# OpenVVC/OpenVVC

Hardware: AMD Instinct MI355X
Metric: decoded frames/sec, full rcn back-end decode step (H2D of the recorded picture + MC incl. BDOF/DMVR/affine-PROF/GPM/CIIP + LMCS + inverse transform + ordered intra pass + deblocking + SAO + ALF/CC-ALF + D2H of refined MVs + wait + per-picture digest + publication to the device DPB), 4K 10-bit RA rec (higher is better)
Workload: dtype u16 samples / int16 coefficients / int32 accumulate

## Files before the change

### openvvc_amd/csrc/kernels_mcx.hip

```cpp
#include "mc_common.hip.h"

#ifndef OV_WPE_MCX
#define OV_WPE_MCX 4
#endif
#if OV_WPE_MCX > 0
#define OV_OCC_MCX __attribute__((amdgpu_waves_per_eu(OV_WPE_MCX)))
#else
#define OV_OCC_MCX
#endif

namespace {

#define XWIN_STRIDE  32
#define XCWIN_STRIDE 20
#define XWIN_ROWS    28
#define XCWIN_ROWS   16
#define BIL_STRIDE   20
#define R_STRIDE     18

__device__ __forceinline__ void clip_mv_dev(int px, int py, int pic_w, int pic_h, int pw, int ph, int &mvx, int &mvy)
{
    mvx = ov_clip3(mvx, -((pw + 3 + px) << 4), (pic_w + 2 - px) << 4);
    mvy = ov_clip3(mvy, -((ph + 3 + py) << 4), (pic_h + 2 - py) << 4);
}

__device__ __forceinline__ void pad_sides(uint16_t *win, int stride, int ww, int wh, int lane)
{
    if (lane < wh) {
        uint16_t *r = win + lane * stride;
        const uint16_t a = r[0], b = r[ww - 1];
        r[-1] = a; r[-2] = a; r[ww] = b; r[ww + 1] = b;
    }
}
__device__ __forceinline__ void pad_rows(uint16_t *win, int stride, int ww, int wh, int lane)
{
    if (lane < ww + 4) {
        uint16_t *c = win + lane - 2;
        const uint16_t a = c[0], b = c[(wh - 1) * stride];
        c[-stride] = a; c[-2 * stride] = a; c[wh * stride] = b; c[(wh + 1) * stride] = b;
    }
}

template <int ND>
__device__ __forceinline__ uint32_t sad_row(const int *a, const int *b, bool odd, uint32_t acc)
{
    uint32_t A[ND + 1], B[ND + 1];
#pragma unroll
    for (int k = 0; k < ND + 1; ++k) { A[k] = (uint32_t)a[k]; B[k] = (uint32_t)b[k]; }
    if (odd) {
#pragma unroll
        for (int k = 0; k < ND; ++k) {
            A[k] = __builtin_amdgcn_alignbit(A[k + 1], A[k], 16);
            B[k] = __builtin_amdgcn_alignbit(B[k + 1], B[k], 16);
        }
    }
#pragma unroll
    for (int k = 0; k < ND; ++k) acc = __builtin_amdgcn_sad_u16(A[k], B[k], acc);
    return acc;
}

__device__ __forceinline__ int div_for_maxq7(int num, int den)
{
    int sign = 0, q = 0;
    if (num < 0) { sign = 1; num = -num; }
    den <<= 3;
    if (num >= den) { num -= den; q++; }
    q <<= 1; den >>= 1;
    if (num >= den) { num -= den; q++; }
    q <<= 1;
    if (num >= (den >> 1)) q++;
    return sign ? -q : q;
}

#define MCX_LDS_WL (2 * XWIN_ROWS * XWIN_STRIDE * 2)
#define MCX_LDS_WC (4 * XCWIN_ROWS * XCWIN_STRIDE * 2)
#define MCX_LDS    (MCX_LDS_WL + MCX_LDS_WC + (2 * 16 * HT_STRIDE + 4 * 8 * CHT_STRIDE) * 2)

template <bool SEARCH_ONLY>
__device__ __forceinline__ void mcx_units(const ovhip_pic &dst, const RefTable &refs, const ovhip_mc_unit *__restrict__ units,
                                          uint32_t n_units, const uint16_t *__restrict__ lmcs_fwd, int32_t *__restrict__ mv_out,
                                          uint32_t wg, char *lds)
{
    uint16_t (*const s_wl)[XWIN_ROWS * XWIN_STRIDE] = reinterpret_cast<uint16_t (*)[XWIN_ROWS * XWIN_STRIDE]>(lds);
    uint16_t (*const s_wc)[2][XCWIN_ROWS * XCWIN_STRIDE] =
        reinterpret_cast<uint16_t (*)[2][XCWIN_ROWS * XCWIN_STRIDE]>(lds + MCX_LDS_WL);
    int16_t *const s_h = reinterpret_cast<int16_t *>(lds + MCX_LDS_WL + MCX_LDS_WC);
    int16_t (*const s_hl)[16 * HT_STRIDE] = reinterpret_cast<int16_t (*)[16 * HT_STRIDE]>(s_h);
    int16_t (*const s_hc)[2][8 * CHT_STRIDE] = reinterpret_cast<int16_t (*)[2][8 * CHT_STRIDE]>(s_h + 2 * 16 * HT_STRIDE);
    int16_t (*const s_x)[24 * BIL_STRIDE] = reinterpret_cast<int16_t (*)[24 * BIL_STRIDE]>(s_h);
    static_assert(2 * 24 * BIL_STRIDE <= 2 * 16 * HT_STRIDE + 4 * 8 * CHT_STRIDE, "bilinear blocks must fit the H tiles");
    uint32_t *const s_ba = reinterpret_cast<uint32_t *>(s_wl[0]);
    uint32_t *const s_bb = s_ba + 256;
    int16_t  *const s_bc = reinterpret_cast<int16_t *>(s_bb + 256);
    static_assert(2 * XWIN_ROWS * XWIN_STRIDE * 2 >= 2 * 1024 + 512, "BDOF terms must fit the luma windows");

    const int lane = threadIdx.x;
    {
    if (wg >= n_units) return;
    const uint32_t bid = ov_xcd_slot(wg, n_units);
    const ovhip_mc_unit u = units[bid];
    const bool dmvr = u.flags & OVHIP_MC_DMVR;
    if (SEARCH_ONLY && !dmvr) return;
    bool use_bdof = u.flags & OVHIP_MC_BDOF;
    const bool do_l = !(u.flags & OVHIP_MC_NO_LUMA), do_c = !(u.flags & OVHIP_MC_NO_CHROMA);
    const int w = u.w, h = u.h, wc = w >> 1, hc = h >> 1;
    const int log2w = 31 - __clz(w), log2wc = log2w - 1;

    int mv[2][2] = { { u.mv0x, u.mv0y }, { u.mv1x, u.mv1y } };
    int ini[2][2] = { { u.mv0x, u.mv0y }, { u.mv1x, u.mv1y } };

    uint16_t *wl[2], *wcp[2][2];
    int offl[2], offc[2];
    {
        const uint16_t *const ry[2]  = { refs.p[u.ref0].y,  refs.p[u.ref1].y };
        const uint16_t *const rcb[2] = { refs.p[u.ref0].cb, refs.p[u.ref1].cb };
        const uint16_t *const rcr[2] = { refs.p[u.ref0].cr, refs.p[u.ref1].cr };
        int lx[2], ly[2], cx[2], cy[2];
#pragma unroll
        for (int l = 0; l < 2; ++l) {
            int ax = mv[l][0], ay = mv[l][1];
            if (dmvr) clip_mv_dev(u.x, u.y, dst.w, dst.h, w, h, ax, ay);
            lx[l] = u.x + (ax >> 4) - 3;        ly[l] = u.y + (ay >> 4) - 3;
            cx[l] = (u.x >> 1) + (ax >> 5) - 1; cy[l] = (u.y >> 1) + (ay >> 5) - 1;
        }
        uint16_t *const lwin[2] = { s_wl[0] + 2 * XWIN_STRIDE + 4, s_wl[1] + 2 * XWIN_STRIDE + 4 };
        uint16_t *const cwin[4] = { s_wc[0][0] + 2 * XCWIN_STRIDE + 4, s_wc[0][1] + 2 * XCWIN_STRIDE + 4,
                                    s_wc[1][0] + 2 * XCWIN_STRIDE + 4, s_wc[1][1] + 2 * XCWIN_STRIDE + 4 };
        stage_unit_windows(dst, ry, rcb, rcr, lx, ly, cx, cy, w, h, 3, do_l, do_c, lane, lwin, XWIN_STRIDE, cwin, XCWIN_STRIDE, offl, offc);
#pragma unroll
        for (int l = 0; l < 2; ++l) {
            wl[l] = lwin[l] + offl[l];
            wcp[0][l] = cwin[l] + offc[l]; wcp[1][l] = cwin[2 + l] + offc[l];
        }
    }
    __syncthreads();

    if (dmvr) {
#pragma unroll
        for (int l = 0; l < 2; ++l) {
            if (do_l) pad_sides(wl[l], XWIN_STRIDE, w + 7, h + 7, lane);
            if (do_c) { pad_sides(wcp[0][l], XCWIN_STRIDE, wc + 3, hc + 3, lane); pad_sides(wcp[1][l], XCWIN_STRIDE, wc + 3, hc + 3, lane); }
        }
        __syncthreads();
#pragma unroll
        for (int l = 0; l < 2; ++l) {
            if (do_l) pad_rows(wl[l], XWIN_STRIDE, w + 7, h + 7, lane);
            if (do_c) { pad_rows(wcp[0][l], XCWIN_STRIDE, wc + 3, hc + 3, lane); pad_rows(wcp[1][l], XCWIN_STRIDE, wc + 3, hc + 3, lane); }
        }
        {
            const int l = lane >= 32, i = lane & 31;
            if (i <= w + 4) {
                const int fx = ini[l][0] & 15, fy = ini[l][1] & 15;
                const uint16_t *src = wl[l] + XWIN_STRIDE + i + 1;
                int16_t *o = s_x[l] + i;
                int tp = 0;
                for (int j = 0; j < h + 5; ++j) {
                    const int a = src[j * XWIN_STRIDE];
                    const int b = __builtin_amdgcn_update_dpp(0, a, 0x130 , 0xf, 0xf, false);
                    const int t = fx ? (__mul24(16 - fx, a) + __mul24(fx, b) + 8) >> 4 : a;
                    if (j && i < w + 4) o[(j - 1) * BIL_STRIDE] = (int16_t)(fy ? (__mul24(16 - fy, tp) + __mul24(fy, t) + 8) >> 4 : tp);
                    tp = t;
                }
            }
        }
        __syncthreads();
        int sad = 0;
        {
            const int k = lane < 25 ? lane : lane - 25, half = lane >= 25;
            if (lane < 50) {
                const int dx = k % 5 - 2, dy = k / 5 - 2;
                const int c0 = 2 + dx, c1 = 2 - dx;
                const bool odd = c0 & 1;
                const int *r0 = reinterpret_cast<const int *>(s_x[0] + (2 + dy) * BIL_STRIDE) + (c0 >> 1);
                const int *r1 = reinterpret_cast<const int *>(s_x[1] + (2 - dy) * BIL_STRIDE) + (c1 >> 1);
                const int nrow = h >> 2;
                uint32_t acc = 0;
                for (int jj = 0; jj < nrow; ++jj) {
                    const int ro = 2 * (half * nrow + jj) * (BIL_STRIDE / 2);
                    if (w == 16) acc = sad_row<8>(r0 + ro, r1 + ro, odd, acc);
                    else         acc = sad_row<4>(r0 + ro, r1 + ro, odd, acc);
                }
// ... 16 lines not shown
            const int s2 = __shfl(sad, max(idx - 5, 0)), s4 = __shfl(sad, min(idx + 5, 24));
            if (abs(dh) != 32 && abs(dv) != 32) {
                const int den_h = s1 + s3 - 2 * s0, den_v = s2 + s4 - 2 * s0;
                if (den_h) dh += (s1 != s0 && s3 != s0) ? div_for_maxq7((s1 - s3) << 4, den_h) : (s1 == s0 ? -8 : 8);
                if (den_v) dv += (s2 != s0 && s4 != s0) ? div_for_maxq7((s2 - s4) << 4, den_v) : (s2 == s0 ? -8 : 8);
            }
            dh = __builtin_amdgcn_readfirstlane(dh); dv = __builtin_amdgcn_readfirstlane(dv);
            mv[0][0] = ov_clip3(mv[0][0] + dh, -(1 << 17), (1 << 17) - 1); mv[0][1] = ov_clip3(mv[0][1] + dv, -(1 << 17), (1 << 17) - 1);
            mv[1][0] = ov_clip3(mv[1][0] - dh, -(1 << 17), (1 << 17) - 1); mv[1][1] = ov_clip3(mv[1][1] - dv, -(1 << 17), (1 << 17) - 1);
        }
        min_cost = __builtin_amdgcn_readfirstlane(min_cost);
        if (use_bdof && min_cost < 2 * w * h) use_bdof = false;
        __syncthreads();
    }
    if (mv_out && lane == 0) {
        int4 o; o.x = mv[0][0]; o.y = mv[0][1]; o.z = mv[1][0]; o.w = mv[1][1];
        *reinterpret_cast<int4 *>(mv_out + 4 * (size_t)bid) = o;
    }
    if (SEARCH_ONLY) return;

    const uint32_t *fvl[2];
    int ldx[2], ldy[2], cdx[2], cdy[2], ext[2][2];
    int fxs[2];
#pragma unroll
    for (int l = 0; l < 2; ++l) {
        int fx = mv[l][0] & 15, fy = mv[l][1] & 15;
        if (u.flags & OVHIP_MC_HPEL_FILT) { if (fx == 8) fx = 16; if (fy == 8) fy = 16; }
        ext[l][0] = fx >= 8; ext[l][1] = fy >= 8;
        fvl[l] = g_taps.luma[fy];
        ldx[l] = (mv[l][0] >> 4) - (ini[l][0] >> 4); ldy[l] = (mv[l][1] >> 4) - (ini[l][1] >> 4);
        cdx[l] = (mv[l][0] >> 5) - (ini[l][0] >> 5); cdy[l] = (mv[l][1] >> 5) - (ini[l][1] >> 5);
        fxs[l] = fx;
    }
    const int hfx = (lane >> 5) ? fxs[1] : fxs[0], hfc = ((lane >> 4) & 1 ? mv[1][0] : mv[0][0]) & 31;
    const uint4 hl_tp = *reinterpret_cast<const uint4 *>(g_taps.luma[hfx]);
    const uint2 hc_tp = *reinterpret_cast<const uint2 *>(g_taps.chroma[hfc]);
    if (do_l) {
        const int l = lane >> 5;
        const int tp[4] = { (int)hl_tp.x, (int)hl_tp.y, (int)hl_tp.z, (int)hl_tp.w };
        const uint16_t *src = s_wl[0] + l * (XWIN_ROWS * XWIN_STRIDE) + (2 + (l ? ldy[1] : ldy[0])) * XWIN_STRIDE;
        const int off = 4 + (l ? offl[1] + ldx[1] : offl[0] + ldx[0]);
        h_pass<8>(src, XWIN_STRIDE, off, h + 7, log2w - 2, 5, lane & 31, tp, hfx == 0, s_hl[0] + l * 16 * HT_STRIDE, HT_STRIDE);
    }
    if (do_c) {
        const int qi = lane >> 4, l = qi & 1;
        const int tp[2] = { (int)hc_tp.x, (int)hc_tp.y };
        const uint16_t *src = s_wc[0][0] + qi * (XCWIN_ROWS * XCWIN_STRIDE) + (2 + (l ? cdy[1] : cdy[0])) * XCWIN_STRIDE;
        const int off = 4 + (l ? offc[1] + cdx[1] : offc[0] + cdx[0]);
        h_pass<4>(src, XCWIN_STRIDE, off, hc + 3, log2wc > 2 ? log2wc - 2 : 0, 4, lane & 15, tp, hfc == 0, s_hc[0][0] + qi * 8 * CHT_STRIDE,
                  CHT_STRIDE);
    }
    __syncthreads();

    if (do_l) {
        int P[2][4];
        v_pass<8>(s_hl[0], HT_STRIDE, log2w, h, fvl[0], lane, P[0]);
        v_pass<8>(s_hl[1], HT_STRIDE, log2w, h, fvl[1], lane, P[1]);
        const bool act = lane < ((h >> 2) << log2w);
        const int x = lane & (w - 1), g = lane >> log2w;
        int out[4];
        if (use_bdof) {
            if (act) {
#pragma unroll
                for (int l = 0; l < 2; ++l)
#pragma unroll
                    for (int j = 0; j < 4; ++j) s_x[l][(4 * g + j + 1) * R_STRIDE + x + 1] = (int16_t)P[l][j];
            }
            const int nring = 2 * (w + 2) + 2 * h;
            for (int t = lane; t < 2 * nring; t += 64) {
                const int l = t >= nring, e = l ? t - nring : t;
                int i, j;
                if (e < w + 2)            { i = e; j = 0; }
                else if (e < 2 * (w + 2)) { i = e - (w + 2); j = h + 1; }
                else if (e < 2 * (w + 2) + h) { i = 0; j = e - 2 * (w + 2) + 1; }
                else                      { i = w + 1; j = e - 2 * (w + 2) - h + 1; }
                const uint16_t *sp = wl[l] + (3 + ldy[l] + j - 1 + ext[l][1]) * XWIN_STRIDE + 3 + ldx[l] + i - 1 + ext[l][0];
                s_x[l][j * R_STRIDE + i] = (int16_t)(*sp << 4);
            }
            __syncthreads();
            int dgx[4], dgy[4];
            if (act) {
                int col[2][6];
#pragma unroll
// ... 34 lines not shown
                        b2 += __builtin_bit_cast(bd_s2, s_bb[idx]);
                        s_dy += s_bc[idx];
                    }
                }
                int s_ax = (unsigned short)a2.x, s_ay = (unsigned short)a2.y, s_xy = b2.x, s_dx = b2.y;
#pragma unroll
                for (int m = 1; m < 4; m <<= 1) {
                    s_ax += __shfl_xor(s_ax, m); s_ay += __shfl_xor(s_ay, m); s_xy += __shfl_xor(s_xy, m);
                    s_dx += __shfl_xor(s_dx, m); s_dy += __shfl_xor(s_dy, m);
                }
                if (s_ax) wx = ov_clip3((s_dx * 4) >> (31 - __clz(s_ax)), -15, 15);
                if (s_ay) {
                    const int x_off = wx ? (wx * s_xy) >> 1 : 0;
                    wy = ov_clip3(((s_dy * 4) - x_off) >> (31 - __clz(s_ay)), -15, 15);
                }
            }
#pragma unroll
            for (int j = 0; j < 4; ++j) out[j] = ov_clip_bd((int)(int16_t)((P[0][j] + P[1][j] + __mul24(wx, dgx[j]) + __mul24(wy, dgy[j]) + 16) >> 5));
        } else {
#pragma unroll
            for (int j = 0; j < 4; ++j) out[j] = ov_clip_bd((P[0][j] + P[1][j] + 16) >> 5);
        }
        if (act) {
            uint16_t *d = dst.y + ov_rowoff(u.y + 4 * g, dst.stride_y) + u.x + x;
#pragma unroll
            for (int j = 0; j < 4; ++j) {
                int v = out[j];
                if ((u.flags & OVHIP_MC_LMCS) && lmcs_fwd) v = lmcs_fwd[v];
                d[j * dst.stride_y] = (uint16_t)v;
            }
        }
    }
    if (do_c) {
        int tvc[2][2];
        load_taps<2>(g_taps.chroma[mv[0][1] & 31], tvc[0]); load_taps<2>(g_taps.chroma[mv[1][1] & 31], tvc[1]);
        if (wc * hc >= 64) chroma_finish<2, true>(u, dst, s_hc[0][0], tvc, lane, log2wc, hc, dst);
        else               chroma_finish<1, true>(u, dst, s_hc[0][0], tvc, lane, log2wc, hc, dst);
    }
    __syncthreads();
    }
}

}


namespace {

#define AWS AFF_WS
#define AHS 12
#define ACS AFF_WS
#define ACHS 8

#ifdef OV_MCA_PHASES
#define OV_MCA_PHASE_UNITS 65536
__device__ unsigned int g_mca_phase[OV_MCA_PHASE_UNITS * 8];
#define OV_APHASE(i) do { __builtin_amdgcn_s_waitcnt(0); const unsigned long long t_ = __builtin_readcyclecounter(); \
                          ph[i] = (unsigned int)(t_ - tprev); tprev = t_; } while (0)
#else
#define OV_APHASE(i) do { } while (0)
#endif

#define MCA_LDS_WIN  (16 * 9 * AWS * 2)
#define MCA_LDS_HT   (16 * 4 * AHS * 2)
#define MCA_LDS_T    (16 * 40 * 2)
#define MCA_LDS_CWIN (2 * 8 * 7 * ACS * 2)
#define MCA_LDS      (MCA_LDS_WIN + MCA_LDS_HT + MCA_LDS_T + MCA_LDS_CWIN + 2 * 8 * 4 * ACHS * 2)

__device__ __forceinline__ void mca_units(const ovhip_pic &dst, const RefTable &refs, const ovhip_aff_unit *__restrict__ units,
                                          uint32_t n_units, const int32_t *__restrict__ side, const uint16_t *__restrict__ lmcs_fwd,
                                          uint32_t wg, char *lds)
{
    uint16_t (*const s_win)[9 * AWS] = reinterpret_cast<uint16_t (*)[9 * AWS]>(lds);
    int16_t  (*const s_ht)[4 * AHS]  = reinterpret_cast<int16_t (*)[4 * AHS]>(lds + MCA_LDS_WIN);
    int16_t  (*const s_t)[40]        = reinterpret_cast<int16_t (*)[40]>(lds + MCA_LDS_WIN + MCA_LDS_HT);
    uint16_t (*const s_cwin)[8][7 * ACS] = reinterpret_cast<uint16_t (*)[8][7 * ACS]>(lds + MCA_LDS_WIN + MCA_LDS_HT + MCA_LDS_T);
    int16_t  (*const s_cht)[8][4 * ACHS] = reinterpret_cast<int16_t (*)[8][4 * ACHS]>(lds + MCA_LDS_WIN + MCA_LDS_HT + MCA_LDS_T + MCA_LDS_CWIN);

    const int lane = threadIdx.x;
    {
    if (wg >= n_units) return;
    const uint32_t bid = ov_xcd_slot(wg, n_units);
#ifdef OV_MCA_PHASES
    unsigned int ph[8] = {}; unsigned long long tprev = __builtin_readcyclecounter();
#endif
    const ovhip_aff_unit u = units[bid];
    OV_APHASE(0);
    const int nsx = u.w >> 2, nsb = nsx * (u.h >> 2), ncx = u.w >> 3, ncb = ncx * (u.h >> 3);
    const bool do_c = !(u.flags & OVHIP_AFF_NO_CHROMA);
    const int4 *mvs = reinterpret_cast<const int4 *>(side + u.side_off);

    const int sb = lane >> 2, c = lane & 3;
    const bool act = sb < nsb;
    const int bx = u.x + 4 * (sb % nsx), by = u.y + 4 * (sb / nsx);
    int4 m = make_int4(0, 0, 0, 0);
    if (act) m = mvs[sb];
    const int cl = lane >> 5, cwi = (lane >> 2) & 7, cblk = cwi & 3, ccomp = cwi >> 2, cc = lane & 3;
    const bool cact = do_c && cblk < ncb && (u.dir & (1 << cl));
    int4 cm = make_int4(0, 0, 0, 0);
    if (do_c && cblk < ncb) cm = mvs[nsb + cblk];
    const int cbx = (u.x >> 1) + 4 * (cblk % ncx), cby = (u.y >> 1) + 4 * (cblk / ncx);
    int coff = 0;

    OV_APHASE(1);

    AffStage<9> st;
    const int rsy = dst.stride_y, rpw = dst.w, rph = dst.h;
    const int lfirst = (u.dir & 1) ? 0 : 1;
    if (act) {
        const int mvx = lfirst ? m.z : m.x, mvy = lfirst ? m.w : m.y;
        st.issue(refs.p[lfirst ? u.ref1 : u.ref0].y, rsy, rpw, rph, bx + (mvx >> 4) - 2, by + (mvy >> 4) - 2, c);
    }
    if (cact) {
        const ovhip_pic &rp = refs.p[cl ? u.ref1 : u.ref0];
        const int mvx = cl ? cm.z : cm.x, mvy = cl ? cm.w : cm.y;
        AffStage<7> cst;
        cst.issue(ccomp ? rp.cr : rp.cb, rp.stride_c, rp.w >> 1, rp.h >> 1, cbx + (mvx >> 5) - 1, cby + (mvy >> 5) - 1, cc);
        coff = cst.park(rp.stride_c, rp.w >> 1, rp.h >> 1, cc, s_cwin[cl][cwi]);
    }
    bool prof[2];
    int pdx[2][4], pdy[2][4];
#pragma unroll
    for (int l = 0; l < 2; ++l) {
        prof[l] = act && (u.dir & (1 << l)) && (u.flags & OVHIP_AFF_PROF) && (u.dir != 3 || ((u.prof_dir >> l) & 1));
        if (prof[l]) {
            const int16_t *pt = reinterpret_cast<const int16_t *>(side + u.prof_off) + 32 * l;
#pragma unroll
            for (int j = 0; j < 4; ++j) { pdx[l][j] = pt[4 * j + c]; pdy[l][j] = pt[16 + 4 * j + c]; }
        }
    }
    OV_APHASE(2);

    int P[2][4] = { { 0, 0, 0, 0 }, { 0, 0, 0, 0 } };
#pragma unroll
    for (int l = 0; l < 2; ++l) {
        const bool on = (u.dir & (1 << l)) && act;
        const int mvx = l ? m.z : m.x, mvy = l ? m.w : m.y;
        int off = 0;
        if (l) __syncthreads();
        if (on) off = st.park(rsy, rpw, rph, c, s_win[sb]);
        if (l == 0 && u.dir == 3 && act)
            st.issue(refs.p[u.ref1].y, rsy, rpw, rph, bx + (m.z >> 4) - 2, by + (m.w >> 4) - 2, c);
        __syncthreads();
        if (on) {
            int tp[3];
            load_taps<3>(g_taps.luma6[mvx & 15], tp);
            for (int r = c; r < 9; r += 4) {
                int d[5], out[4];
                load_row_at<6>(s_win[sb] + r * AWS, off, d);
                fir4<6>(d, tp, out);
#pragma unroll
                for (int o = 0; o < 4; ++o) s_ht[sb][o * AHS + r] = (int16_t)(out[o] >> (OV_BD - 8));
            }
        }
        if (l == 0 && cact) {
            const int cmvx = cl ? cm.z : cm.x;
            int tp[2];
            load_taps<2>(g_taps.chroma[cmvx & 31], tp);
            for (int r = cc; r < 7; r += 4) {
                int d[4], out[4];
                load_row_at<4>(s_cwin[cl][cwi] + r * ACS, coff, d);
                fir4<4>(d, tp, out);
#pragma unroll
                for (int o = 0; o < 4; ++o) s_cht[cl][cwi][o * ACHS + r] = (int16_t)(out[o] >> (OV_BD - 8));
            }
        }
        __syncthreads();
        if (on) {
            int tp[3], d[5];
            load_taps<3>(g_taps.luma6[mvy & 15], tp);
            const int *q = reinterpret_cast<const int *>(s_ht[sb] + c * AHS);
#pragma unroll
            for (int j = 0; j < 5; ++j) d[j] = q[j];
            fir4<6>(d, tp, P[l]);
#pragma unroll
            for (int o = 0; o < 4; ++o) P[l][o] >>= 6;
        }
        if (prof[l]) {
            const int ex = (mvx & 15) >> 3, ey = (mvy & 15) >> 3;
            const uint16_t *wp = s_win[sb] + (1 + ey) * AWS + off + 1 + ex;
            prof_fill(s_t[sb], c, P[l], [wp](int i, int j) { return (int)wp[j * AWS + i]; });
        }
        __syncthreads();
        if (prof[l]) prof_refine(s_t[sb], c, pdx[l], pdy[l], P[l]);
    }
    OV_APHASE(4);
    if (act) {
        const Combine cmb = mc_combine_of(BiMode{ ((u.ident_l >> sb) & 1) ? 2 : u.dir, u.w0, u.w1 });
        uint16_t *d = dst.y + ov_rowoff(by, dst.stride_y) + bx + c;
#pragma unroll
        for (int j = 0; j < 4; ++j) {
            int v = mc_combine(cmb, P[0][j], P[1][j]);
            if ((u.flags & OVHIP_AFF_LMCS) && lmcs_fwd) v = lmcs_fwd[v];
            d[j * dst.stride_y] = (uint16_t)v;
        }
    }
    OV_APHASE(5);
    if (do_c && lane < 32 && cblk < ncb) {
        int Pc[2][4] = { { 0, 0, 0, 0 }, { 0, 0, 0, 0 } };
#pragma unroll
        for (int l = 0; l < 2; ++l) {
            if (!(u.dir & (1 << l))) continue;
            const int mvy = l ? cm.w : cm.y;
            int tp[2], d[4];
            load_taps<2>(g_taps.chroma[mvy & 31], tp);
            const int *q = reinterpret_cast<const int *>(s_cht[l][cwi] + cc * ACHS);
#pragma unroll
            for (int j = 0; j < 4; ++j) d[j] = q[j];
            fir4<4>(d, tp, Pc[l]);
#pragma unroll
            for (int o = 0; o < 4; ++o) Pc[l][o] >>= 6;
        }
        const Combine cmb = mc_combine_of(BiMode{ ((u.ident_c >> cblk) & 1) ? 2 : u.dir, u.w0, u.w1 });
        uint16_t *d = (ccomp ? dst.cr : dst.cb) + ov_rowoff(cby, dst.stride_c) + cbx + cc;
#pragma unroll
        for (int j = 0; j < 4; ++j) d[j * dst.stride_c] = (uint16_t)mc_combine(cmb, Pc[0][j], Pc[1][j]);
    }
    __syncthreads();
#ifdef OV_MCA_PHASES
    OV_APHASE(6);
    if (lane == 0 && bid < OV_MCA_PHASE_UNITS) {
#pragma unroll
        for (int i = 0; i < 7; ++i) g_mca_phase[bid * 8 + i] = ph[i];
        g_mca_phase[bid * 8 + 7] = 1;
    }
#endif
    }
}

__global__ __launch_bounds__(64) OV_OCC_MCX void k_mcx(ovhip_pic dst, RefTable refs, const ovhip_mc_unit *__restrict__ units,
                                             uint32_t n_units, const uint16_t *__restrict__ lmcs_fwd, int32_t *__restrict__ mv_out)
{
    __shared__ __attribute__((aligned(16))) char lds[MCX_LDS];
    mcx_units<false>(dst, refs, units, n_units, lmcs_fwd, mv_out, blockIdx.x, lds);
}

__global__ __launch_bounds__(64) OV_OCC_MCX void k_dmvr_search(ovhip_pic geom, RefTable refs, const ovhip_mc_unit *__restrict__ units,
                                                     uint32_t n_units, int32_t *__restrict__ mv_out)
{
    __shared__ __attribute__((aligned(16))) char lds[MCX_LDS];
    mcx_units<true>(geom, refs, units, n_units, nullptr, mv_out, blockIdx.x, lds);
}

__global__ __launch_bounds__(64) OV_OCC_MCX void k_mca(ovhip_pic dst, RefTable refs, const ovhip_aff_unit *__restrict__ units,
                                             uint32_t n_units, const int32_t *__restrict__ side, const uint16_t *__restrict__ lmcs_fwd)
{
    __shared__ __attribute__((aligned(16))) char lds[MCA_LDS];
    mca_units(dst, refs, units, n_units, side, lmcs_fwd, blockIdx.x, lds);
}

__global__ __launch_bounds__(64) OV_OCC_MCX void k_mcxa(ovhip_pic dst, RefTable refs, const ovhip_mc_unit *__restrict__ xunits, uint32_t n_x,
                                              int32_t *__restrict__ mv_out, const ovhip_aff_unit *__restrict__ aunits, uint32_t n_a,
                                              const int32_t *__restrict__ side, const uint16_t *__restrict__ lmcs_fwd)
{
    __shared__ __attribute__((aligned(16))) char lds[MCX_LDS > MCA_LDS ? MCX_LDS : MCA_LDS];
    if (blockIdx.x < n_a) mca_units(dst, refs, aunits, n_a, side, lmcs_fwd, blockIdx.x, lds);
    else                  mcx_units<false>(dst, refs, xunits, n_x, lmcs_fwd, mv_out, blockIdx.x - n_a, lds);
}

}

#ifdef OV_MCA_PHASES
extern "C" int ovhip_debug_mca_phases(unsigned int *out )
{
    return hipMemcpyFromSymbol(out, HIP_SYMBOL(g_mca_phase), sizeof(unsigned int) * OV_MCA_PHASE_UNITS * 8) == hipSuccess ? OVHIP_OK : OVHIP_ELAUNCH;
}
#endif

extern "C" int ovhip_mcx_launch(ovhip_ctx *ctx, const ovhip_pic *dst, const ovhip_pic *refs, uint32_t n_refs,
                                const ovhip_mc_unit *d_units, uint32_t n_units, const uint16_t *d_lmcs_fwd_lut,
                                int32_t *d_mv_out)
{
    if (!ctx || !dst) return OVHIP_EINVAL;
    OV_DEVICE(ctx);
    if (!n_units) return OVHIP_OK;
    if (!d_units) return ov_fail(ctx, OVHIP_EINVAL, "ovhip_mcx_launch: null units", hipSuccess);
    RefTable t;
    if (int e = ref_table(ctx, &t, refs, n_refs, dst, "ovhip_mcx_launch")) return e;
    hipLaunchKernelGGL(k_mcx, dim3(n_units), dim3(64), 0, ctx->stream, *dst, t, d_units, n_units, d_lmcs_fwd_lut, d_mv_out);
    OV_LAUNCH_CHECK(ctx, "k_mcx");
    return OVHIP_OK;
}

extern "C" int ovhip_dmvr_search_launch(ovhip_ctx *ctx, const ovhip_pic *geom, const ovhip_pic *refs, uint32_t n_refs,
                                        const ovhip_mc_unit *d_units, uint32_t n_units, int32_t *d_mv_out)
{
    if (!ctx || !geom) return OVHIP_EINVAL;
    OV_DEVICE(ctx);
// ... 42 lines not shown
```

### openvvc_amd/csrc/kernels_output.hip

```cpp
#include <hip/hip_runtime.h>
#include <stdint.h>
#include <stdlib.h>
#include <string.h>
#include "ovvc_hip.h"
#include "ovvc_common.hip.h"
#include "ovvc_dpb_priv.h"
#include "ovvc_reduce_priv.h"

namespace {

struct OutGeom {
    const uint16_t *src[3]; int stride[3], w[3], h[3];
    size_t first_sample[3], first_row[3];
    size_t samples, rows;
};

static bool out_geom(int32_t w, int32_t h, const ovhip_window *win, const ovhip_pic *pic, OutGeom &g)
{
    const int l = win ? win->offset_lft : 0, r = win ? win->offset_rgt : 0, a = win ? win->offset_abv : 0, b = win ? win->offset_blw : 0;
    g.samples = 0; g.rows = 0;
    for (int c = 0; c < 3; ++c) {
        const int sh = c ? 0 : 1, pw = c ? w >> 1 : w, ph = c ? h >> 1 : h;
        g.w[c] = pw - ((l + r) << sh); g.h[c] = ph - ((a + b) << sh);
        if (g.w[c] <= 0 || g.h[c] <= 0) return false;
// ... 92 lines not shown
__device__ __forceinline__ void md5_digests(const uint32_t *w, int nd, uint32_t h[4])
{
    h[0] = 0x67452301u; h[1] = 0xefcdab89u; h[2] = 0x98badcfeu; h[3] = 0x10325476u;
    uint32_t m[16];
    int d = 0;
    for (; d + 4 <= nd; d += 4) {
#pragma unroll
        for (int i = 0; i < 16; ++i) m[i] = w[4 * d + i];
        md5_block(h, m);
    }
    const int rem = nd - d;
#pragma unroll
    for (int i = 0; i < 16; ++i) m[i] = i < 4 * rem ? w[4 * d + i] : (i == 4 * rem ? 0x80u : 0u);
    const uint64_t bits = (uint64_t)nd * 128;
    m[14] = (uint32_t)bits; m[15] = (uint32_t)(bits >> 32);
    md5_block(h, m);
}

__device__ __forceinline__ uint32_t mix_fin(uint32_t h)
{
    h ^= h >> 16; h *= 0x85ebca6bu; h ^= h >> 13; h *= 0xc2b2ae35u; h ^= h >> 16;
    return h;
}
#define MIX_STEP(hj, w) (hj) = ((hj) ^ (w)) * 0x01000193u
__device__ __forceinline__ void mix_begin(uint32_t h[4], uint32_t tag)
{
    h[0] = 0x67452301u ^ tag; h[1] = 0xefcdab89u; h[2] = 0x98badcfeu; h[3] = 0x10325476u;
}
__device__ __forceinline__ void mix_end(uint32_t h[4])
{
    h[0] = mix_fin(h[0]); h[1] = mix_fin(h[1]); h[2] = mix_fin(h[2]); h[3] = mix_fin(h[3]);
    h[0] += h[1]; h[2] += h[3]; h[0] += h[2]; h[1] += h[0]; h[2] += h[0]; h[3] += h[0];
}
__device__ __forceinline__ void mix_samples(const uint16_t *src, int n, uint32_t h[4])
{
    mix_begin(h, (uint32_t)n);
    int s = 0;
    if (((uintptr_t)src & 15) == 0) {
        const uint4 *s128 = reinterpret_cast<const uint4 *>(src);
        for (; s + 8 <= n; s += 8) {
            const uint4 v = s128[s >> 3];
            MIX_STEP(h[0], v.x); MIX_STEP(h[1], v.y); MIX_STEP(h[2], v.z); MIX_STEP(h[3], v.w);
        }
    } else {
        for (; s + 8 <= n; s += 8) {
#pragma unroll
            for (int j = 0; j < 4; ++j) MIX_STEP(h[j], (uint32_t)src[s + 2 * j] | ((uint32_t)src[s + 2 * j + 1] << 16));
        }
    }
    for (int j = 0; s < n; s += 2, ++j) MIX_STEP(h[j], (uint32_t)src[s] | (s + 1 < n ? (uint32_t)src[s + 1] << 16 : 0u));
    mix_end(h);
}
__device__ __forceinline__ void mix_digests(const uint32_t *w, int nd, uint32_t h[4])
{
    mix_begin(h, (uint32_t)nd);
    for (int d = 0; d < nd; ++d) { MIX_STEP(h[0], w[4 * d]); MIX_STEP(h[1], w[4 * d + 1]); MIX_STEP(h[2], w[4 * d + 2]); MIX_STEP(h[3], w[4 * d + 3]); }
    mix_end(h);
}

__global__ __launch_bounds__(64) void k_output_row_md5(OutGeom g, uint8_t *__restrict__ digests)
{
    const size_t row = (size_t)blockIdx.x * 64 + threadIdx.x;
    if (row >= g.rows) return;
    const int c = row >= g.first_row[2] ? 2 : (row >= g.first_row[1] ? 1 : 0);
    uint32_t h[4];
    md5_samples(g.src[c] + (row - g.first_row[c]) * (size_t)g.stride[c], g.w[c], h);
    uint32_t *o = reinterpret_cast<uint32_t *>(digests + row * 16);
    o[0] = h[0]; o[1] = h[1]; o[2] = h[2]; o[3] = h[3];
}

#define DG_SEG   256
#define DG_BAND  8
#define DG_MAXSEG 64
#define DG_NT    128
__global__ __launch_bounds__(DG_NT) void k_output_tree_md5(OutGeom g, uint32_t nb0, uint32_t nb1, uint8_t *__restrict__ digests)
{
    __shared__ uint32_t s_d0[DG_BAND * DG_MAXSEG * 4];
    __shared__ uint32_t s_d1[DG_BAND * 4];
    const uint32_t band = blockIdx.x;
    const int c = band >= nb0 + nb1 ? 2 : (band >= nb0 ? 1 : 0);
    const int r0 = (int)(band - (c == 2 ? nb0 + nb1 : (c == 1 ? nb0 : 0))) * DG_BAND;
    const int nrows = min(DG_BAND, g.h[c] - r0), w = g.w[c], nseg = (w + DG_SEG - 1) / DG_SEG;
    const int tid = threadIdx.x;
    for (int i = tid; i < nrows * nseg; i += DG_NT) {
        const int r = i / nseg, k = i - r * nseg;
        uint32_t h[4];
        mix_samples(g.src[c] + (size_t)(r0 + r) * g.stride[c] + k * DG_SEG, min(DG_SEG, w - k * DG_SEG), h);
        uint32_t *o = s_d0 + (r * DG_MAXSEG + k) * 4;
        o[0] = h[0]; o[1] = h[1]; o[2] = h[2]; o[3] = h[3];
    }
    __syncthreads();
    if (tid < nrows) {
        uint32_t h[4];
        mix_digests(s_d0 + tid * DG_MAXSEG * 4, nseg, h);
        s_d1[4 * tid] = h[0]; s_d1[4 * tid + 1] = h[1]; s_d1[4 * tid + 2] = h[2]; s_d1[4 * tid + 3] = h[3];
    }
    __syncthreads();
    if (tid == 0) {
        uint32_t h[4];
        mix_digests(s_d1, nrows, h);
        uint32_t *o = reinterpret_cast<uint32_t *>(digests + (size_t)band * 16);
        o[0] = h[0]; o[1] = h[1]; o[2] = h[2]; o[3] = h[3];
    }
}

}

extern "C" size_t ovhip_output_bytes(int32_t w, int32_t h, const ovhip_window *win)
{
    OutGeom g;
    if (w <= 0 || h <= 0 || (w & 1) || (h & 1) || !out_geom(w, h, win, nullptr, g)) return 0;
    return g.samples * sizeof(uint16_t);
}

extern "C" size_t ovhip_output_rows(int32_t w, int32_t h, const ovhip_window *win)
{
    OutGeom g;
    if (w <= 0 || h <= 0 || (w & 1) || (h & 1) || !out_geom(w, h, win, nullptr, g)) return 0;
    return g.rows;
}

extern "C" int ovhip_output_pack_launch(ovhip_ctx *ctx, const ovhip_pic *pic, const ovhip_window *win, uint16_t *d_out)
// ... 184 lines not shown
```

Measured before the change: 3589.

## Shrink MC LDS footprint, stage chroma via registers, parallelize digest lanes

The combined MC kernel now overlays the chroma windows and H tiles onto the dead luma windows and raises the waves-per-EU hint, so more work-groups fit per CU. Chroma reference fetches are issued into registers early and parked in LDS only after luma is done, and affine chroma loads are deferred to overlap with luma filtering. The output digest kernel splits each segment hash across four lanes using DPP exchange, with twice the threads per block. The price is extra barriers, more register pressure from the in-flight chroma loads, and a tail-handling path in the digest whose ordering must still match the previous hash.

```diff
diff --git a/openvvc_amd/csrc/kernels_mcx.hip b/openvvc_amd/csrc/kernels_mcx.hip
--- a/openvvc_amd/csrc/kernels_mcx.hip
+++ b/openvvc_amd/csrc/kernels_mcx.hip
@@ -1,7 +1,7 @@
 #include "mc_common.hip.h"
 
 #ifndef OV_WPE_MCX
-#define OV_WPE_MCX 4
+#define OV_WPE_MCX 6
 #endif
 #if OV_WPE_MCX > 0
 #define OV_OCC_MCX __attribute__((amdgpu_waves_per_eu(OV_WPE_MCX)))
@@ -11,7 +11,9 @@
 
 namespace {
 
+#ifndef XWIN_STRIDE
 #define XWIN_STRIDE  32
+#endif
 #define XCWIN_STRIDE 20
 #define XWIN_ROWS    28
 #define XCWIN_ROWS   16
@@ -74,7 +76,12 @@
 
 #define MCX_LDS_WL (2 * XWIN_ROWS * XWIN_STRIDE * 2)
 #define MCX_LDS_WC (4 * XCWIN_ROWS * XCWIN_STRIDE * 2)
-#define MCX_LDS    (MCX_LDS_WL + MCX_LDS_WC + (2 * 16 * HT_STRIDE + 4 * 8 * CHT_STRIDE) * 2)
+#define MCX_LDS_T  (2 * 24 * BIL_STRIDE * 2)
+#define MCX_LDS    (MCX_LDS_WL + MCX_LDS_T)
+#define MC_UNIT_LDS_STEP 6400
+static_assert(MCX_LDS <= MC_UNIT_LDS_STEP, "a refined unit must stay under the 24-per-CU step of LDS");
+static_assert(MCX_LDS_WC + 4 * 8 * CHT_STRIDE * 2 <= MCX_LDS_WL, "chroma windows + H tiles must fit the (dead) luma windows");
+static_assert(2 * 16 * HT_STRIDE * 2 <= MCX_LDS_T && 2 * 18 * R_STRIDE * 2 <= MCX_LDS_T, "luma H tiles / BDOF R tiles must fit the tile region");
 
 template <bool SEARCH_ONLY>
 __device__ __forceinline__ void mcx_units(const ovhip_pic &dst, const RefTable &refs, const ovhip_mc_unit *__restrict__ units,
@@ -82,13 +89,11 @@
                                           uint32_t wg, char *lds)
 {
     uint16_t (*const s_wl)[XWIN_ROWS * XWIN_STRIDE] = reinterpret_cast<uint16_t (*)[XWIN_ROWS * XWIN_STRIDE]>(lds);
-    uint16_t (*const s_wc)[2][XCWIN_ROWS * XCWIN_STRIDE] =
-        reinterpret_cast<uint16_t (*)[2][XCWIN_ROWS * XCWIN_STRIDE]>(lds + MCX_LDS_WL);
-    int16_t *const s_h = reinterpret_cast<int16_t *>(lds + MCX_LDS_WL + MCX_LDS_WC);
+    uint16_t (*const s_wc)[2][XCWIN_ROWS * XCWIN_STRIDE] = reinterpret_cast<uint16_t (*)[2][XCWIN_ROWS * XCWIN_STRIDE]>(lds);
+    int16_t (*const s_hc)[2][8 * CHT_STRIDE] = reinterpret_cast<int16_t (*)[2][8 * CHT_STRIDE]>(lds + MCX_LDS_WC);
+    int16_t *const s_h = reinterpret_cast<int16_t *>(lds + MCX_LDS_WL);
     int16_t (*const s_hl)[16 * HT_STRIDE] = reinterpret_cast<int16_t (*)[16 * HT_STRIDE]>(s_h);
-    int16_t (*const s_hc)[2][8 * CHT_STRIDE] = reinterpret_cast<int16_t (*)[2][8 * CHT_STRIDE]>(s_h + 2 * 16 * HT_STRIDE);
     int16_t (*const s_x)[24 * BIL_STRIDE] = reinterpret_cast<int16_t (*)[24 * BIL_STRIDE]>(s_h);
-    static_assert(2 * 24 * BIL_STRIDE <= 2 * 16 * HT_STRIDE + 4 * 8 * CHT_STRIDE, "bilinear blocks must fit the H tiles");
     uint32_t *const s_ba = reinterpret_cast<uint32_t *>(s_wl[0]);
     uint32_t *const s_bb = s_ba + 256;
     int16_t  *const s_bc = reinterpret_cast<int16_t *>(s_bb + 256);
@@ -109,44 +114,41 @@
     int mv[2][2] = { { u.mv0x, u.mv0y }, { u.mv1x, u.mv1y } };
     int ini[2][2] = { { u.mv0x, u.mv0y }, { u.mv1x, u.mv1y } };
 
-    uint16_t *wl[2], *wcp[2][2];
+    uint16_t *wl[2];
     int offl[2], offc[2];
-    {
-        const uint16_t *const ry[2]  = { refs.p[u.ref0].y,  refs.p[u.ref1].y };
-        const uint16_t *const rcb[2] = { refs.p[u.ref0].cb, refs.p[u.ref1].cb };
-        const uint16_t *const rcr[2] = { refs.p[u.ref0].cr, refs.p[u.ref1].cr };
-        int lx[2], ly[2], cx[2], cy[2];
+    const uint16_t *const ry[2]  = { refs.p[u.ref0].y,  refs.p[u.ref1].y };
+    const uint16_t *const rcb[2] = { refs.p[u.ref0].cb, refs.p[u.ref1].cb };
+    const uint16_t *const rcr[2] = { refs.p[u.ref0].cr, refs.p[u.ref1].cr };
+    uint16_t *const lwin[2] = { s_wl[0] + 2 * XWIN_STRIDE + 4, s_wl[1] + 2 * XWIN_STRIDE + 4 };
+    uint16_t *const cwin[4] = { s_wc[0][0] + 2 * XCWIN_STRIDE + 4, s_wc[0][1] + 2 * XCWIN_STRIDE + 4,
+                                s_wc[1][0] + 2 * XCWIN_STRIDE + 4, s_wc[1][1] + 2 * XCWIN_STRIDE + 4 };
+    int lx[2], ly[2], cx[2], cy[2];
+#pragma unroll
+    for (int l = 0; l < 2; ++l) {
+        int ax = mv[l][0], ay = mv[l][1];
+        if (dmvr) clip_mv_dev(u.x, u.y, dst.w, dst.h, w, h, ax, ay);
+        lx[l] = u.x + (ax >> 4) - 3;        ly[l] = u.y + (ay >> 4) - 3;
+        cx[l] = (u.x >> 1) + (ax >> 5) - 1; cy[l] = (u.y >> 1) + (ay >> 5) - 1;
+    }
+    ChromaStage sc[2][2];
+    const bool c_regs = !SEARCH_ONLY && do_c && !((dst.stride_y | dst.stride_c | dst.w | (dst.w >> 1)) & 3)
+                        && (ChromaStage::interior(cx[0], cy[0], wc + 3, hc + 3, dst.w >> 1, dst.h >> 1)
+                            & ChromaStage::interior(cx[1], cy[1], wc + 3, hc + 3, dst.w >> 1, dst.h >> 1));
+    if (c_regs) {
 #pragma unroll
         for (int l = 0; l < 2; ++l) {
-            int ax = mv[l][0], ay = mv[l][1];
-            if (dmvr) clip_mv_dev(u.x, u.y, dst.w, dst.h, w, h, ax, ay);
-            lx[l] = u.x + (ax >> 4) - 3;        ly[l] = u.y + (ay >> 4) - 3;
-            cx[l] = (u.x >> 1) + (ax >> 5) - 1; cy[l] = (u.y >> 1) + (ay >> 5) - 1;
-        }
-        uint16_t *const lwin[2] = { s_wl[0] + 2 * XWIN_STRIDE + 4, s_wl[1] + 2 * XWIN_STRIDE + 4 };
-        uint16_t *const cwin[4] = { s_wc[0][0] + 2 * XCWIN_STRIDE + 4, s_wc[0][1] + 2 * XCWIN_STRIDE + 4,
-                                    s_wc[1][0] + 2 * XCWIN_STRIDE + 4, s_wc[1][1] + 2 * XCWIN_STRIDE + 4 };
-        stage_unit_windows(dst, ry, rcb, rcr, lx, ly, cx, cy, w, h, 3, do_l, do_c, lane, lwin, XWIN_STRIDE, cwin, XCWIN_STRIDE, offl, offc);
-#pragma unroll
-        for (int l = 0; l < 2; ++l) {
-            wl[l] = lwin[l] + offl[l];
-            wcp[0][l] = cwin[l] + offc[l]; wcp[1][l] = cwin[2 + l] + offc[l];
-        }
-    }
+            sc[0][l].issue_fast(rcb[l], dst.stride_c, cx[l], cy[l], wc + 3, hc + 3, lane);
+            sc[1][l].issue_fast(rcr[l], dst.stride_c, cx[l], cy[l], wc + 3, hc + 3, lane);
+        }
+    }
+    stage_unit_windows(dst, ry, rcb, rcr, lx, ly, cx, cy, w, h, 3, do_l || dmvr, false, lane, lwin, XWIN_STRIDE, cwin, XCWIN_STRIDE, offl, offc);
+    wl[0] = lwin[0] + offl[0]; wl[1] = lwin[1] + offl[1];
     __syncthreads();
 
     if (dmvr) {
-#pragma unroll
-        for (int l = 0; l < 2; ++l) {
-            if (do_l) pad_sides(wl[l], XWIN_STRIDE, w + 7, h + 7, lane);
-            if (do_c) { pad_sides(wcp[0][l], XCWIN_STRIDE, wc + 3, hc + 3, lane); pad_sides(wcp[1][l], XCWIN_STRIDE, wc + 3, hc + 3, lane); }
-        }
-        __syncthreads();
-#pragma unroll
-        for (int l = 0; l < 2; ++l) {
-            if (do_l) pad_rows(wl[l], XWIN_STRIDE, w + 7, h + 7, lane);
-            if (do_c) { pad_rows(wcp[0][l], XCWIN_STRIDE, wc + 3, hc + 3, lane); pad_rows(wcp[1][l], XCWIN_STRIDE, wc + 3, hc + 3, lane); }
-        }
+        pad_sides(wl[0], XWIN_STRIDE, w + 7, h + 7, lane); pad_sides(wl[1], XWIN_STRIDE, w + 7, h + 7, lane);
+        __syncthreads();
+        pad_rows(wl[0], XWIN_STRIDE, w + 7, h + 7, lane); pad_rows(wl[1], XWIN_STRIDE, w + 7, h + 7, lane);
         {
             const int l = lane >= 32, i = lane & 31;
             if (i <= w + 4) {
@@ -229,23 +231,14 @@
         cdx[l] = (mv[l][0] >> 5) - (ini[l][0] >> 5); cdy[l] = (mv[l][1] >> 5) - (ini[l][1] >> 5);
         fxs[l] = fx;
     }
-    const int hfx = (lane >> 5) ? fxs[1] : fxs[0], hfc = ((lane >> 4) & 1 ? mv[1][0] : mv[0][0]) & 31;
+    const int hfx = (lane >> 5) ? fxs[1] : fxs[0];
     const uint4 hl_tp = *reinterpret_cast<const uint4 *>(g_taps.luma[hfx]);
-    const uint2 hc_tp = *reinterpret_cast<const uint2 *>(g_taps.chroma[hfc]);
     if (do_l) {
         const int l = lane >> 5;
         const int tp[4] = { (int)hl_tp.x, (int)hl_tp.y, (int)hl_tp.z, (int)hl_tp.w };
         const uint16_t *src = s_wl[0] + l * (XWIN_ROWS * XWIN_STRIDE) + (2 + (l ? ldy[1] : ldy[0])) * XWIN_STRIDE;
         const int off = 4 + (l ? offl[1] + ldx[1] : offl[0] + ldx[0]);
         h_pass<8>(src, XWIN_STRIDE, off, h + 7, log2w - 2, 5, lane & 31, tp, hfx == 0, s_hl[0] + l * 16 * HT_STRIDE, HT_STRIDE);
-    }
-    if (do_c) {
-        const int qi = lane >> 4, l = qi & 1;
-        const int tp[2] = { (int)hc_tp.x, (int)hc_tp.y };
-        const uint16_t *src = s_wc[0][0] + qi * (XCWIN_ROWS * XCWIN_STRIDE) + (2 + (l ? cdy[1] : cdy[0])) * XCWIN_STRIDE;
-        const int off = 4 + (l ? offc[1] + cdx[1] : offc[0] + cdx[0]);
-        h_pass<4>(src, XCWIN_STRIDE, off, hc + 3, log2wc > 2 ? log2wc - 2 : 0, 4, lane & 15, tp, hfc == 0, s_hc[0][0] + qi * 8 * CHT_STRIDE,
-                  CHT_STRIDE);
     }
     __syncthreads();
 
@@ -346,6 +339,42 @@
         }
     }
     if (do_c) {
+        __syncthreads();
+        if (c_regs) {
+#pragma unroll
+            for (int l = 0; l < 2; ++l) {
+                sc[0][l].park<false>(cwin[l], XCWIN_STRIDE, wc + 3, hc + 3, lane);
+                sc[1][l].park<false>(cwin[2 + l], XCWIN_STRIDE, wc + 3, hc + 3, lane);
+                offc[l] = sc[0][l].off;
+            }
+        } else {
+            int none[2];
+            stage_unit_windows(dst, ry, rcb, rcr, lx, ly, cx, cy, w, h, 3, false, true, lane, lwin, XWIN_STRIDE, cwin, XCWIN_STRIDE, none, offc);
+        }
+        __syncthreads();
+        if (dmvr) {
+#pragma unroll
+            for (int l = 0; l < 2; ++l) {
+                pad_sides(cwin[l] + offc[l], XCWIN_STRIDE, wc + 3, hc + 3, lane); pad_sides(cwin[2 + l] + offc[l], XCWIN_STRIDE, wc + 3, hc + 3, lane);
+            }
+            __syncthreads();
+#pragma unroll
+            for (int l = 0; l < 2; ++l) {
+                pad_rows(cwin[l] + offc[l], XCWIN_STRIDE, wc + 3, hc + 3, lane); pad_rows(cwin[2 + l] + offc[l], XCWIN_STRIDE, wc + 3, hc + 3, lane);
+            }
+            __syncthreads();
+        }
+        {
+            const int qi = lane >> 4, l = qi & 1;
+            const int hfc = (l ? mv[1][0] : mv[0][0]) & 31;
+            const uint2 hc_tp = *reinterpret_cast<const uint2 *>(g_taps.chroma[hfc]);
+            const int tp[2] = { (int)hc_tp.x, (int)hc_tp.y };
+            const uint16_t *src = s_wc[0][0] + qi * (XCWIN_ROWS * XCWIN_STRIDE) + (2 + (l ? cdy[1] : cdy[0])) * XCWIN_STRIDE;
+            const int off = 4 + (l ? offc[1] + cdx[1] : offc[0] + cdx[0]);
+            h_pass<4>(src, XCWIN_STRIDE, off, hc + 3, log2wc > 2 ? log2wc - 2 : 0, 4, lane & 15, tp, hfc == 0, s_hc[0][0] + qi * 8 * CHT_STRIDE,
+                      CHT_STRIDE);
+        }
+        __syncthreads();
         int tvc[2][2];
         load_taps<2>(g_taps.chroma[mv[0][1] & 31], tvc[0]); load_taps<2>(g_taps.chroma[mv[1][1] & 31], tvc[1]);
         if (wc * hc >= 64) chroma_finish<2, true>(u, dst, s_hc[0][0], tvc, lane, log2wc, hc, dst);
@@ -378,7 +407,10 @@
 #define MCA_LDS_HT   (16 * 4 * AHS * 2)
 #define MCA_LDS_T    (16 * 40 * 2)
 #define MCA_LDS_CWIN (2 * 8 * 7 * ACS * 2)
-#define MCA_LDS      (MCA_LDS_WIN + MCA_LDS_HT + MCA_LDS_T + MCA_LDS_CWIN + 2 * 8 * 4 * ACHS * 2)
+#define MCA_LDS_CHT  (2 * 8 * 4 * ACHS * 2)
+#define MCA_LDS      (MCA_LDS_WIN + MCA_LDS_HT + MCA_LDS_T)
+static_assert(MCA_LDS <= MC_UNIT_LDS_STEP, "an affine unit must stay under the 24-per-CU step of LDS");
+static_assert(MCA_LDS_CWIN + MCA_LDS_CHT <= MCA_LDS, "chroma windows + H tiles must fit the (dead) luma tiles");
 
 __device__ __forceinline__ void mca_units(const ovhip_pic &dst, const RefTable &refs, const ovhip_aff_unit *__restrict__ units,
                                           uint32_t n_units, const int32_t *__restrict__ side, const uint16_t *__restrict__ lmcs_fwd,
@@ -387,8 +419,8 @@
     uint16_t (*const s_win)[9 * AWS] = reinterpret_cast<uint16_t (*)[9 * AWS]>(lds);
     int16_t  (*const s_ht)[4 * AHS]  = reinterpret_cast<int16_t (*)[4 * AHS]>(lds + MCA_LDS_WIN);
     int16_t  (*const s_t)[40]        = reinterpret_cast<int16_t (*)[40]>(lds + MCA_LDS_WIN + MCA_LDS_HT);
-    uint16_t (*const s_cwin)[8][7 * ACS] = reinterpret_cast<uint16_t (*)[8][7 * ACS]>(lds + MCA_LDS_WIN + MCA_LDS_HT + MCA_LDS_T);
-    int16_t  (*const s_cht)[8][4 * ACHS] = reinterpret_cast<int16_t (*)[8][4 * ACHS]>(lds + MCA_LDS_WIN + MCA_LDS_HT + MCA_LDS_T + MCA_LDS_CWIN);
+    uint16_t (*const s_cwin)[8][7 * ACS] = reinterpret_cast<uint16_t (*)[8][7 * ACS]>(lds);
+    int16_t  (*const s_cht)[8][4 * ACHS] = reinterpret_cast<int16_t (*)[8][4 * ACHS]>(lds + MCA_LDS_CWIN);
 
     const int lane = threadIdx.x;
     {
@@ -424,22 +456,16 @@
         const int mvx = lfirst ? m.z : m.x, mvy = lfirst ? m.w : m.y;
         st.issue(refs.p[lfirst ? u.ref1 : u.ref0].y, rsy, rpw, rph, bx + (mvx >> 4) - 2, by + (mvy >> 4) - 2, c);
     }
-    if (cact) {
-        const ovhip_pic &rp = refs.p[cl ? u.ref1 : u.ref0];
-        const int mvx = cl ? cm.z : cm.x, mvy = cl ? cm.w : cm.y;
-        AffStage<7> cst;
-        cst.issue(ccomp ? rp.cr : rp.cb, rp.stride_c, rp.w >> 1, rp.h >> 1, cbx + (mvx >> 5) - 1, cby + (mvy >> 5) - 1, cc);
-        coff = cst.park(rp.stride_c, rp.w >> 1, rp.h >> 1, cc, s_cwin[cl][cwi]);
-    }
+    AffStage<7> cst;
     bool prof[2];
-    int pdx[2][4], pdy[2][4];
+    int pd[2][4];
 #pragma unroll
     for (int l = 0; l < 2; ++l) {
         prof[l] = act && (u.dir & (1 << l)) && (u.flags & OVHIP_AFF_PROF) && (u.dir != 3 || ((u.prof_dir >> l) & 1));
         if (prof[l]) {
             const int16_t *pt = reinterpret_cast<const int16_t *>(side + u.prof_off) + 32 * l;
 #pragma unroll
-            for (int j = 0; j < 4; ++j) { pdx[l][j] = pt[4 * j + c]; pdy[l][j] = pt[16 + 4 * j + c]; }
+            for (int j = 0; j < 4; ++j) pd[l][j] = (int)((uint32_t)(uint16_t)pt[4 * j + c] | ((uint32_t)(uint16_t)pt[16 + 4 * j + c] << 16));
         }
     }
     OV_APHASE(2);
@@ -454,6 +480,11 @@
         if (on) off = st.park(rsy, rpw, rph, c, s_win[sb]);
         if (l == 0 && u.dir == 3 && act)
             st.issue(refs.p[u.ref1].y, rsy, rpw, rph, bx + (m.z >> 4) - 2, by + (m.w >> 4) - 2, c);
+        if (l == 1 && cact) {
+            const ovhip_pic &rp = refs.p[cl ? u.ref1 : u.ref0];
+            const int cmvx = cl ? cm.z : cm.x, cmvy = cl ? cm.w : cm.y;
+            cst.issue(ccomp ? rp.cr : rp.cb, rp.stride_c, rp.w >> 1, rp.h >> 1, cbx + (cmvx >> 5) - 1, cby + (cmvy >> 5) - 1, cc);
+        }
         __syncthreads();
         if (on) {
             int tp[3];
@@ -466,7 +497,50 @@
                 for (int o = 0; o < 4; ++o) s_ht[sb][o * AHS + r] = (int16_t)(out[o] >> (OV_BD - 8));
             }
         }
-        if (l == 0 && cact) {
+        __syncthreads();
+        if (on) {
+            int tp[3], d[5];
+            load_taps<3>(g_taps.luma6[mvy & 15], tp);
+            const int *q = reinterpret_cast<const int *>(s_ht[sb] + c * AHS);
+#pragma unroll
+            for (int j = 0; j < 5; ++j) d[j] = q[j];
+            fir4<6>(d, tp, P[l]);
+#pragma unroll
+            for (int o = 0; o < 4; ++o) P[l][o] >>= 6;
+        }
+        if (prof[l]) {
+            const int ex = (mvx & 15) >> 3, ey = (mvy & 15) >> 3;
+            const uint16_t *wp = s_win[sb] + (1 + ey) * AWS + off + 1 + ex;
+            prof_fill(s_t[sb], c, P[l], [wp](int i, int j) { return (int)wp[j * AWS + i]; });
+        }
+        __syncthreads();
+        if (prof[l]) {
+            int pdx[4], pdy[4];
+#pragma unroll
+            for (int j = 0; j < 4; ++j) { pdx[j] = (int16_t)pd[l][j]; pdy[j] = pd[l][j] >> 16; }
+            prof_refine(s_t[sb], c, pdx, pdy, P[l]);
+        }
+    }
+    OV_APHASE(4);
+    if (act) {
+        const Combine cmb = mc_combine_of(BiMode{ ((u.ident_l >> sb) & 1) ? 2 : u.dir, u.w0, u.w1 });
+        uint16_t *d = dst.y + ov_rowoff(by, dst.stride_y) + bx + c;
+#pragma unroll
+        for (int j = 0; j < 4; ++j) {
+            int v = mc_combine(cmb, P[0][j], P[1][j]);
+            if ((u.flags & OVHIP_AFF_LMCS) && lmcs_fwd) v = lmcs_fwd[v];
+            d[j * dst.stride_y] = (uint16_t)v;
+        }
+    }
+    OV_APHASE(5);
+    if (do_c) {
+        __syncthreads();
+        if (cact) {
+            const ovhip_pic &rp = refs.p[cl ? u.ref1 : u.ref0];
+            coff = cst.park(rp.stride_c, rp.w >> 1, rp.h >> 1, cc, s_cwin[cl][cwi]);
+        }
+        __syncthreads();
+        if (cact) {
             const int cmvx = cl ? cm.z : cm.x;
             int tp[2];
             load_taps<2>(g_taps.chroma[cmvx & 31], tp);
@@ -479,36 +553,7 @@
             }
         }
         __syncthreads();
-        if (on) {
-            int tp[3], d[5];
-            load_taps<3>(g_taps.luma6[mvy & 15], tp);
-            const int *q = reinterpret_cast<const int *>(s_ht[sb] + c * AHS);
-#pragma unroll
-            for (int j = 0; j < 5; ++j) d[j] = q[j];
-            fir4<6>(d, tp, P[l]);
-#pragma unroll
-            for (int o = 0; o < 4; ++o) P[l][o] >>= 6;
-        }
-        if (prof[l]) {
-            const int ex = (mvx & 15) >> 3, ey = (mvy & 15) >> 3;
-            const uint16_t *wp = s_win[sb] + (1 + ey) * AWS + off + 1 + ex;
-            prof_fill(s_t[sb], c, P[l], [wp](int i, int j) { return (int)wp[j * AWS + i]; });
-        }
-        __syncthreads();
-        if (prof[l]) prof_refine(s_t[sb], c, pdx[l], pdy[l], P[l]);
-    }
-    OV_APHASE(4);
-    if (act) {
-        const Combine cmb = mc_combine_of(BiMode{ ((u.ident_l >> sb) & 1) ? 2 : u.dir, u.w0, u.w1 });
-        uint16_t *d = dst.y + ov_rowoff(by, dst.stride_y) + bx + c;
-#pragma unroll
-        for (int j = 0; j < 4; ++j) {
-            int v = mc_combine(cmb, P[0][j], P[1][j]);
-            if ((u.flags & OVHIP_AFF_LMCS) && lmcs_fwd) v = lmcs_fwd[v];
-            d[j * dst.stride_y] = (uint16_t)v;
-        }
-    }
-    OV_APHASE(5);
+    }
     if (do_c && lane < 32 && cblk < ncb) {
         int Pc[2][4] = { { 0, 0, 0, 0 }, { 0, 0, 0, 0 } };
 #pragma unroll
@@ -567,6 +612,7 @@
                                               const int32_t *__restrict__ side, const uint16_t *__restrict__ lmcs_fwd)
 {
     __shared__ __attribute__((aligned(16))) char lds[MCX_LDS > MCA_LDS ? MCX_LDS : MCA_LDS];
+    static_assert(sizeof(lds) <= MC_UNIT_LDS_STEP, "k_mcxa must stay under the 24-per-CU step of LDS");
     if (blockIdx.x < n_a) mca_units(dst, refs, aunits, n_a, side, lmcs_fwd, blockIdx.x, lds);
     else                  mcx_units<false>(dst, refs, xunits, n_x, lmcs_fwd, mv_out, blockIdx.x - n_a, lds);
 }
diff --git a/openvvc_amd/csrc/kernels_output.hip b/openvvc_amd/csrc/kernels_output.hip
--- a/openvvc_amd/csrc/kernels_output.hip
+++ b/openvvc_amd/csrc/kernels_output.hip
@@ -148,24 +148,38 @@
     h[0] = mix_fin(h[0]); h[1] = mix_fin(h[1]); h[2] = mix_fin(h[2]); h[3] = mix_fin(h[3]);
     h[0] += h[1]; h[2] += h[3]; h[0] += h[2]; h[1] += h[0]; h[2] += h[0]; h[3] += h[0];
 }
-__device__ __forceinline__ void mix_samples(const uint16_t *src, int n, uint32_t h[4])
-{
-    mix_begin(h, (uint32_t)n);
-    int s = 0;
-    if (((uintptr_t)src & 15) == 0) {
-        const uint4 *s128 = reinterpret_cast<const uint4 *>(src);
-        for (; s + 8 <= n; s += 8) {
-            const uint4 v = s128[s >> 3];
-            MIX_STEP(h[0], v.x); MIX_STEP(h[1], v.y); MIX_STEP(h[2], v.z); MIX_STEP(h[3], v.w);
+__device__ __forceinline__ void mix_samples_quad(const uint16_t *src, int n, int j, uint32_t h[4])
+{
+    uint32_t hj = j == 0 ? 0x67452301u ^ (uint32_t)n : (j == 1 ? 0xefcdab89u : (j == 2 ? 0x98badcfeu : 0x10325476u));
+    const int nfull = n >> 1;
+    int k = j;
+    if (((uintptr_t)src & 3) == 0) {
+        const uint32_t *p = reinterpret_cast<const uint32_t *>(src);
+        for (; k + 28 < nfull; k += 32) {
+            uint32_t w[8];
+#pragma unroll
+            for (int t = 0; t < 8; ++t) w[t] = p[k + 4 * t];
+#pragma unroll
+            for (int t = 0; t < 8; ++t) MIX_STEP(hj, w[t]);
         }
+        for (; k < nfull; k += 4) MIX_STEP(hj, p[k]);
     } else {
-        for (; s + 8 <= n; s += 8) {
-#pragma unroll
-            for (int j = 0; j < 4; ++j) MIX_STEP(h[j], (uint32_t)src[s + 2 * j] | ((uint32_t)src[s + 2 * j + 1] << 16));
+        for (; k + 12 < nfull; k += 16) {
+            uint32_t w[4];
+#pragma unroll
+            for (int t = 0; t < 4; ++t) w[t] = (uint32_t)src[2 * (k + 4 * t)] | ((uint32_t)src[2 * (k + 4 * t) + 1] << 16);
+#pragma unroll
+            for (int t = 0; t < 4; ++t) MIX_STEP(hj, w[t]);
         }
-    }
-    for (int j = 0; s < n; s += 2, ++j) MIX_STEP(h[j], (uint32_t)src[s] | (s + 1 < n ? (uint32_t)src[s + 1] << 16 : 0u));
-    mix_end(h);
+        for (; k < nfull; k += 4) MIX_STEP(hj, (uint32_t)src[2 * k] | ((uint32_t)src[2 * k + 1] << 16));
+    }
+    if ((n & 1) && k == nfull) MIX_STEP(hj, (uint32_t)src[n - 1]);
+    hj = mix_fin(hj);
+    h[0] = (uint32_t)__builtin_amdgcn_update_dpp(0, (int)hj, 0x00 , 0xf, 0xf, false);
+    h[1] = (uint32_t)__builtin_amdgcn_update_dpp(0, (int)hj, 0x55 , 0xf, 0xf, false);
+    h[2] = (uint32_t)__builtin_amdgcn_update_dpp(0, (int)hj, 0xaa , 0xf, 0xf, false);
+    h[3] = (uint32_t)__builtin_amdgcn_update_dpp(0, (int)hj, 0xff , 0xf, 0xf, false);
+    h[0] += h[1]; h[2] += h[3]; h[0] += h[2]; h[1] += h[0]; h[2] += h[0]; h[3] += h[0];
 }
 __device__ __forceinline__ void mix_digests(const uint32_t *w, int nd, uint32_t h[4])
 {
@@ -188,7 +202,7 @@
 #define DG_SEG   256
 #define DG_BAND  8
 #define DG_MAXSEG 64
-#define DG_NT    128
+#define DG_NT    256
 __global__ __launch_bounds__(DG_NT) void k_output_tree_md5(OutGeom g, uint32_t nb0, uint32_t nb1, uint8_t *__restrict__ digests)
 {
     __shared__ uint32_t s_d0[DG_BAND * DG_MAXSEG * 4];
@@ -198,12 +212,12 @@
     const int r0 = (int)(band - (c == 2 ? nb0 + nb1 : (c == 1 ? nb0 : 0))) * DG_BAND;
     const int nrows = min(DG_BAND, g.h[c] - r0), w = g.w[c], nseg = (w + DG_SEG - 1) / DG_SEG;
     const int tid = threadIdx.x;
-    for (int i = tid; i < nrows * nseg; i += DG_NT) {
+    const int j = tid & 3;
+    for (int i = tid >> 2; i < nrows * nseg; i += DG_NT / 4) {
         const int r = i / nseg, k = i - r * nseg;
         uint32_t h[4];
-        mix_samples(g.src[c] + (size_t)(r0 + r) * g.stride[c] + k * DG_SEG, min(DG_SEG, w - k * DG_SEG), h);
-        uint32_t *o = s_d0 + (r * DG_MAXSEG + k) * 4;
-        o[0] = h[0]; o[1] = h[1]; o[2] = h[2]; o[3] = h[3];
+        mix_samples_quad(g.src[c] + (size_t)(r0 + r) * g.stride[c] + k * DG_SEG, min(DG_SEG, w - k * DG_SEG), j, h);
+        s_d0[(r * DG_MAXSEG + k) * 4 + j] = j == 0 ? h[0] : (j == 1 ? h[1] : (j == 2 ? h[2] : h[3]));
     }
     __syncthreads();
     if (tid < nrows) {
```

After: 3682, median of 6. +2.6%, better.
